# Shreyas2409/Rust-Image-Transform

Measured on AMD Instinct MI355X. Metric: transform MPix/s (decode+resize+encode) 4096²→512² WebP q80; 1/2/4/8 GPU, higher is better.
Workload: dtype u8

## Files before the change

rust-image-transform_amd/csrc/ik_inflate.h:

```cpp
#pragma once
#include <stdint.h>

#if defined(__HIPCC__) || defined(__HIP__)
#include <hip/hip_runtime.h>
#define IK_HD __host__ __device__ __forceinline__
#define IK_HD_COLD __host__ __device__ __attribute__((noinline))
#define IK_UNROLL _Pragma("unroll")
#else
#define IK_UNROLL
#define IK_HD inline
#define IK_HD_COLD inline
#endif

#if defined(__HIP_DEVICE_COMPILE__)
#define IK_GLOBAL __attribute__((address_space(1)))
#else
#define IK_GLOBAL
#endif

namespace ik {
namespace infl {

constexpr int kWindow = 32768;

// ... 391 lines not shown
        if (q < 0) return -1;
    }
    return -1;
}


constexpr int kCanonWords = 48;
struct CanonRegs {
    uint32_t lpk[8], dpk[8];
};
IK_HD void pack_limits(const uint32_t (&lim)[15], uint32_t (&pk)[8]) {
    for (int k = 0; k < 7; ++k)
        pk[k] = ((lim[2 * k] - 1u) & 0xFFFFu) | (((lim[2 * k + 1] - 1u) & 0xFFFFu) << 16);
    pk[7] = (lim[14] - 1u) & 0xFFFFu;
}

IK_HD uint32_t rev32(uint32_t v) {
#if defined(__HIP_DEVICE_COMPILE__)
    return __builtin_bitreverse32(v);
#else
    v = ((v >> 1) & 0x55555555u) | ((v & 0x55555555u) << 1);
    v = ((v >> 2) & 0x33333333u) | ((v & 0x33333333u) << 2);
    v = ((v >> 4) & 0x0F0F0F0Fu) | ((v & 0x0F0F0F0Fu) << 4);
    v = ((v >> 8) & 0x00FF00FFu) | ((v & 0x00FF00FFu) << 8);
    return (v >> 16) | (v << 16);
#endif
}

template <class Mem>
IK_HD uint8_t cm_byte(const Mem& m, int i) { return (uint8_t)(m[32 + (i >> 2)] >> (8 * (i & 3))); }

constexpr uint32_t kTokRaw = 0x4000u, kTokMatch = 0x8000u, kTokTable = 0xFFFFu, kTokPad = 0xFFFEu;
constexpr uint32_t kTokTableLen = 128;
constexpr uint32_t kTokSlack = 16;

IK_HD uint32_t tok_capacity(uint64_t bits, bool exact) {
    uint64_t c = (exact ? bits : bits / 4) + 2 * kTokTableLen + 64;
    if (c > 0x7FFFFFF0ull) c = 0x7FFFFFF0ull;
    return (uint32_t)((c + 7) & ~7ull);
}

struct TokOut {
    IK_GLOBAL uint16_t* p;
    uint64_t p0 = 0, p1 = 0, q0 = 0, q1 = 0;
    uint32_t ppos = 0, qpos = 0;
    int npend = 0;
    IK_HD void group(uint32_t pos, uint64_t lo, uint64_t hi) {
        if (npend == 0) {
            p0 = lo;
            p1 = hi;
            ppos = pos;
        } else {
            q0 = lo;
            q1 = hi;
            qpos = pos;
        }
        ++npend;
    }
    IK_HD void store1(uint32_t pos, uint64_t lo, uint64_t hi) {
#if defined(__HIP_DEVICE_COMPILE__)
        typedef uint32_t u4 __attribute__((ext_vector_type(4)));
        const u4 v = {(uint32_t)lo, (uint32_t)(lo >> 32), (uint32_t)hi, (uint32_t)(hi >> 32)};
        *reinterpret_cast<IK_GLOBAL u4*>(p + pos) = v;
#else
        for (int k = 0; k < 4; ++k) {
            p[pos + k] = (uint16_t)(lo >> (16 * k));
// ... 405 lines not shown
```

rust-image-transform_amd/csrc/ik_png.hip:

```cpp
#include <algorithm>
#include <cstdlib>
#include <cstring>
#include <type_traits>

#include "ik_crc.h"
#include "ik_inflate.h"
#include "ik_internal.h"
#include "ik_png.h"
#include "ik_png_wave.h"
#include "ik_unfilter.h"

namespace ik {

__device__ __forceinline__ void raise_priority() { __builtin_amdgcn_s_setprio(3); }

typedef __attribute__((address_space(3))) uint32_t lds_word;
struct FindWin {
    const IK_GLOBAL uint32_t* W;
    uint64_t wend;
    lds_word* win;
    uint32_t r0;
    __device__ void fetch(uint64_t base) {
        if (base + 32 > wend + 64) {
            for (int k = 0; k < 32; ++k) win[64 * k] = base + k < wend ? W[base + k] : 0u;
// ... 307 lines not shown
    }
    __device__ uint64_t operator()(uint32_t pos) {
        const uint32_t d = (pos >> 5) - wi;
        asm("" : "+v"(b0), "+v"(b1), "+v"(b2), "+v"(b3), "+v"(p0), "+v"(p1));
        const uint32_t n0 = d == 0 ? b0 : d == 1 ? b1 : b2;
        const uint32_t n1 = d == 0 ? b1 : d == 1 ? b2 : b3;
        const uint32_t n2 = d == 0 ? b2 : d == 1 ? b3 : p0;
        const uint32_t n3 = d == 0 ? b3 : d == 1 ? p0 : p1;
        b0 = n0;
        b1 = n1;
        b2 = n2;
        b3 = n3;
        wi += d;
        p0 = w[wi + 4];
        p1 = w[wi + 5];
        const uint32_t sh = pos & 31u;
        return ((uint64_t)__builtin_amdgcn_alignbit(b2, b1, sh) << 32) | __builtin_amdgcn_alignbit(b1, b0, sh);
    }
};
struct WaveGlobalWin {
    const IK_GLOBAL uint32_t* w;
    __device__ uint64_t operator()(uint64_t pos) const {
        const uint64_t wi = pos >> 5;
        const uint32_t sh = (uint32_t)(pos & 31u);
        const uint32_t a = w[wi], b = w[wi + 1], c = w[wi + 2];
        const uint32_t lo = __builtin_amdgcn_alignbit(b, a, sh), hi = __builtin_amdgcn_alignbit(c, b, sh);
        return ((uint64_t)hi << 32) | lo;
    }
};

struct WaveOut {
    IK_GLOBAL uint16_t* p;
    uint32_t cap;
    uint32_t n = 0;
    uint64_t g0 = 0, g1 = 0;
    __device__ void reset() { n = 0; g0 = 0; g1 = 0; }
    __device__ void mark(uint32_t, uint32_t) const {}
    __device__ void store(uint32_t g) const {
        if (g + 8u > cap) return;
        typedef uint32_t u4 __attribute__((ext_vector_type(4)));
        const u4 q = {(uint32_t)g0, (uint32_t)(g0 >> 32), (uint32_t)g1, (uint32_t)(g1 >> 32)};
        *reinterpret_cast<IK_GLOBAL u4*>(p + g) = q;
    }
    __device__ void put4(uint32_t a, uint32_t b, uint32_t c, uint32_t d, uint32_t k) {
        uint64_t T = (uint64_t)(a & 0xFFFFu) | ((uint64_t)(b & 0xFFFFu) << 16) | ((uint64_t)(c & 0xFFFFu) << 32) |
                     ((uint64_t)d << 48);
        T &= k >= 4u ? ~0ull : (1ull << (16u * k)) - 1ull;
        const uint32_t off = 16u * (n & 7u);
        const uint64_t lo_part = T << (off & 63u), hi_part = (T >> 1) >> (63u - (off & 63u));
        g0 |= off < 64u ? lo_part : 0ull;
        g1 |= off < 64u ? hi_part : lo_part;
        const uint64_t carry = off > 64u ? hi_part : 0ull;
        const uint32_t n2 = n + k;
        const bool done = ((n2 ^ n) & ~7u) != 0u;
        if (done) store(n & ~7u);
        g0 = done ? carry : g0;
        g1 = done ? 0ull : g1;
        n = n2;
    }
    __device__ void finish() {
        if (n & 7u) {
            constexpr uint64_t P = 0xFFFEFFFEFFFEFFFEull;
            const uint32_t off = 16u * (n & 7u);
            if (off < 64u) {
                g0 |= P << off;
                g1 |= P;
            } else {
                g1 |= P << (off - 64u);
            }
            store(n & ~7u);
        }
    }
};

__device__ __forceinline__ uint64_t shfl_up_u64(uint64_t v, int d) {
    const uint32_t lo = (uint32_t)__shfl_up((int)(uint32_t)v, d, 64), hi = (uint32_t)__shfl_up((int)(uint32_t)(v >> 32), d, 64);
    return ((uint64_t)hi << 32) | lo;
}
__device__ __forceinline__ uint64_t readlane_u64(uint64_t v, int l) {
    const uint32_t lo = (uint32_t)__builtin_amdgcn_readlane((int)(uint32_t)v, l);
    const uint32_t hi = (uint32_t)__builtin_amdgcn_readlane((int)(uint32_t)(v >> 32), l);
    return ((uint64_t)hi << 32) | lo;
}
__device__ __forceinline__ uint64_t wave_sum_u64(uint64_t v) {
#pragma unroll
    for (int o = 32; o >= 1; o >>= 1) {
        const uint32_t lo = (uint32_t)__shfl_xor((int)(uint32_t)v, o, 64), hi = (uint32_t)__shfl_xor((int)(uint32_t)(v >> 32), o, 64);
        v += ((uint64_t)hi << 32) | lo;
    }
    return v;
}

__device__ __forceinline__ uint32_t lane_rank(unsigned long long m) {
    return __builtin_amdgcn_mbcnt_hi((uint32_t)(m >> 32), __builtin_amdgcn_mbcnt_lo((uint32_t)m, 0u));
}

__device__ bool wave_code_build(const uint8_t* lens, int n, bool is_dist, bool fixed, wave::Code& C, uint16_t* syms) {
    const int lane = threadIdx.x;
    uint32_t cnt[16];
#pragma unroll
    for (int l = 0; l < 16; ++l) cnt[l] = 0;
    for (int c0 = 0; c0 < n; c0 += 64) {
        const int sy = c0 + lane;
// ... 414 lines not shown
        }
        if (bfinal) {
            final_block = 1;
            status = stop == ~0ull ? infl::kLaneOk : infl::kLaneMismatch;
            break;
        }
    }
    const uint32_t tsteps = (uint32_t)wave_sum_u64(steps);
    if (lane == 0) {
        infl::LaneResult r{};
        r.end_bit = p;
        r.out_len = total;
        r.ntok = (uint32_t)written;
        r.status = status;
        r.final_block = final_block;
        r.iters = tsteps;
        r.kcycles = (uint32_t)((clock64() - c0) >> 10);
        r.blocks = nblocks;
        r.pieces = npieces;
        r.kc_setup = (uint32_t)(ck_setup >> 10);
        r.units = nunits;
        res[t] = r;
#ifdef IK_WAVE_PROF
        wprof[0] = clock64() - c0;
        wprof[7] = 1;
        for (int k = 0; k < 8; ++k) atomicAdd(&g_wave_prof[k], (unsigned long long)wprof[k]);
#endif
    }
}

constexpr int kXRing = 2048;
constexpr int kXCap = 1024;
constexpr int kXNear = kXRing - kXCap;
using infl::kTokMatch;
using infl::kTokPad;
using infl::kTokRaw;
using infl::kTokTable;
using infl::kTokTableLen;

constexpr uint32_t kX8Tok = 512;
constexpr int kXFar = 64;
constexpr int kXPieces = 192;

#ifdef IK_EXP_PROF
__device__ unsigned long long g_exp_prof[8];
hipError_t png_exp_prof_read(unsigned long long* out) {
    hipError_t e = hipMemcpyFromSymbol(out, HIP_SYMBOL(g_exp_prof), sizeof(g_exp_prof));
    unsigned long long z[8] = {};
    if (e == hipSuccess) e = hipMemcpyToSymbol(HIP_SYMBOL(g_exp_prof), z, sizeof(z));
    return e;
}
#define IK_XP(k) do { const uint64_t _t = clock64(); xprof[k] += _t - xt; xt = _t; } while (0)
#else
#define IK_XP(k) ((void)0)
#endif

template <bool TAB>
__global__ __launch_bounds__(64) void k_png_expand8(const PngImgDev* imgs, const PngLaneDev* lanes, int nlanes,
                                                    const uint16_t* tok, int* status, const uint2* pieces,
                                                    const uint2* units, const uint32_t* ulane, PngMarks mk_out) {
    raise_priority();
    __shared__ __attribute__((aligned(16))) uint16_t s_ring[kXRing];
    __shared__ uint32_t s_tab[TAB ? 64 : 1];
    __shared__ uint32_t s_pb[kXPieces], s_ps[kXPieces];
    __shared__ uint32_t s_fo[kXFar], s_fd[kXFar], s_fc[kXFar];
    constexpr uint32_t M = kXRing - 1;
    typedef uint32_t u4 __attribute__((ext_vector_type(4)));
    const int li = blockIdx.x;
    if (li >= nlanes) return;
    const int x = threadIdx.x;
    const uint64_t c0 = clock64();
    const PngLaneDev L = lanes[units ? (int)ulane[li] : li];
    const PngImgDev I = imgs[L.img];
    const IK_GLOBAL uint16_t* T = (const IK_GLOBAL uint16_t*)(tok + L.tbase);
    IK_GLOBAL uint16_t* const U = (IK_GLOBAL uint16_t*)I.u16;
    int64_t ob = L.obase, oe = L.obase + (int64_t)L.out_len;
    uint32_t ntok = L.ntok;
    const uint32_t np = pieces ? L.npieces : 0u;
    const IK_GLOBAL uint2* P = (const IK_GLOBAL uint2*)(pieces + (pieces ? L.pbase : 0));
    uint32_t pf = 0, t0 = 0;
    if (units) {
        const IK_GLOBAL uint2* R = (const IK_GLOBAL uint2*)(units + L.pbase);
        const uint32_t b = (uint32_t)li - L.ubase;
        const uint2 r0 = make_uint2(R[b].x, R[b].y);
        const bool last = b + 1 >= L.nunits;
        uint2 r1 = make_uint2(np, (uint32_t)L.out_len);
        if (!last) r1 = make_uint2(R[b + 1].x, R[b + 1].y);
        pf = r0.x;
        t0 = P[pf].y;
        ntok = r1.x < np ? P[r1.x].y : L.ntok;
        ob = L.obase + (int64_t)r0.y;
        oe = L.obase + (int64_t)r1.y;
    }
    if (np) {
        for (uint32_t k = (uint32_t)x; pf + k < np && k < (uint32_t)kXPieces; k += 64) {
            s_pb[k] = P[pf + k].x;
            s_ps[k] = P[pf + k].y;
        }
        __syncthreads();
// ... 5 lines not shown
        pc_base = piece_base(pf);
        pn_start = pf + 1 < np ? piece_start(pf + 1) : 0xFFFFFFFFu;
    }
    uint32_t t = t0;
    int64_t cnt = 0;
    bool have_tab = false, bad = false;
    auto load8 = [&](uint32_t a) -> u4 {
        const uint32_t i = a + 8u * (uint32_t)x;
        if (i >= ntok) return u4{0xFFFEFFFEu, 0xFFFEFFFEu, 0xFFFEFFFEu, 0xFFFEFFFEu};
        if (!np) return *(const IK_GLOBAL u4*)(T + i);
        while (i >= pn_start) {
            ++kc;
            pc_base = piece_base(kc);
            pc_start = pn_start;
            pn_start = kc + 1 < np ? piece_start(kc + 1) : 0xFFFFFFFFu;
        }
        return *(const IK_GLOBAL u4*)(T + pc_base + (i - pc_start));
    };
    u4 w = load8(t0 & ~7u);
#ifdef IK_EXP_PROF
    uint64_t xprof[8] = {0, 0, 0, 0, 0, 0, 0, 0}, xt = clock64();
#endif
    while (t < ntok) {
        IK_XP(5);
        const uint32_t a = t & ~7u, i0 = a + 8u * (uint32_t)x;
        uint32_t u[8];
#pragma unroll
        for (int k = 0; k < 4; ++k) {
            u[2 * k] = w[k] & 0xFFFFu;
            u[2 * k + 1] = w[k] >> 16;
        }
        IK_XP(6);
        uint32_t end = a + kX8Tok < ntok ? a + kX8Tok : ntok;
        if constexpr (TAB) {
            int ft = 8;
#pragma unroll
            for (int k = 7; k >= 0; --k)
                if (i0 + k >= t && i0 + k < ntok && u[k] == kTokTable) ft = k;
            const unsigned long long tl = __ballot(ft < 8);
            if (tl) {
                const int l = __builtin_ctzll(tl);
                const uint32_t e = a + 8u * (uint32_t)l + (uint32_t)__builtin_amdgcn_readlane(ft, l);
                if (e == t) {
                    const uint32_t tt = (t + 8) & ~7u;
                    if (tt + kTokTableLen > ntok) { bad = true; break; }
                    s_tab[x] = ((const IK_GLOBAL uint32_t*)(T + tt))[x];
                    have_tab = true;
                    t = tt + kTokTableLen;
                    w = load8(t & ~7u);
                    __syncthreads();
                    continue;
                }
                end = e;
            }
        }
        {
            const uint32_t q = end - 1u;
            const bool mine = q >= t && (q >> 3) == (i0 >> 3);
            const uint32_t wq = w[(q >> 1) & 3u];
            const uint32_t uq = (q & 1u) ? wq >> 16 : wq & 0xFFFFu;
            if (__ballot(mine && (uq & 0xFF00u) == kTokMatch)) --end;
        }
        if (end <= t) { bad = true; break; }
        const uint32_t nx = (uint32_t)__shfl_down((int)u[0], 1, 64);
        const uint32_t pv = (uint32_t)__shfl_up((int)u[7], 1, 64);
        uint32_t len[8], val[8], lit = 0;
        uint32_t bd = 0;
#pragma unroll
        for (int k = 0; k < 8; ++k) {
            const uint32_t idx = i0 + k;
            const uint32_t prev = k ? u[k - 1] : pv, nxt = k < 7 ? u[k + 1] : nx;
            const uint32_t v = u[k];
            const bool start = (idx >= t) & (idx < end) & !((idx > t) & ((prev & 0xFF00u) == kTokMatch));
            const bool raw = (v & 0xFF00u) == kTokRaw, mt = (v & 0xFF00u) == kTokMatch, pad = v == kTokPad;
            const bool rk = TAB && v < 256u;
            const bool isl = raw | rk;
            len[k] = !start ? 0u : isl ? 1u : mt ? (v & 0xFFu) + 3u : 0u;
            uint32_t lv = v & 0xFFu;
            if constexpr (TAB) {
                if (start & rk) lv = (s_tab[v >> 2] >> (8 * (v & 3u))) & 0xFFu;
                bd |= (uint32_t)(start & rk & !have_tab);
            }
            val[k] = isl ? lv : nxt + 1u;
            lit |= (uint32_t)isl << k;
            bd |= (uint32_t)(start & !(isl | mt | pad));
        }
        if (__ballot(bd != 0u)) { bad = true; break; }
        uint32_t off[8], tot;
        for (;;) {
            uint32_t sum = 0;
#pragma unroll
            for (int k = 0; k < 8; ++k) sum += len[k];
            const uint32_t incl = wave_incl_scan_dpp(sum);
            tot = (uint32_t)__builtin_amdgcn_readlane((int)incl, 63);
            off[0] = incl - sum;
#pragma unroll
            for (int k = 1; k < 8; ++k) off[k] = off[k - 1] + len[k - 1];
            if (tot <= (uint32_t)kXCap) break;
            int fk = 8;
#pragma unroll
            for (int k = 7; k >= 0; --k)
                if (len[k] && off[k] + len[k] > (uint32_t)kXCap) fk = k;
            const unsigned long long ov = __ballot(fk < 8);
            const int l = __builtin_ctzll(ov);
            end = a + 8u * (uint32_t)l + (uint32_t)__builtin_amdgcn_readlane(fk, l);
#pragma unroll
            for (int k = 0; k < 8; ++k)
                if (i0 + k >= end) len[k] = 0;
        }
        IK_XP(1);
        const uint32_t t2 = end;
        const u4 wn = t2 < ntok ? load8(t2 & ~7u) : u4{0, 0, 0, 0};
        const uint32_t gb = (uint32_t)(ob + cnt);
#pragma unroll
        for (int k = 0; k < 8; ++k)
            if (len[k] && ((lit >> k) & 1u)) s_ring[(gb + off[k]) & M] = (uint16_t)val[k];
        uint32_t fcnt = 0, flen = 0;
#pragma unroll
        for (int k = 0; k < 8; ++k) {
            const bool fk = len[k] != 0u && !((lit >> k) & 1u) && val[k] > (uint32_t)kXNear;
            fcnt += fk ? 1u : 0u;
            flen += fk ? len[k] : 0u;
        }
        const uint32_t fp = fcnt | (flen << 16), fincl = wave_incl_scan_dpp(fp);
        const uint32_t ftot = (uint32_t)__builtin_amdgcn_readlane((int)fincl, 63);
        const uint32_t F = ftot & 0xFFFFu, FT = ftot >> 16;
        const bool flat = F != 0u && F <= (uint32_t)kXFar;
        if (flat) {
            uint32_t ri = (fincl - fp) & 0xFFFFu, rc = (fincl - fp) >> 16;
#pragma unroll
            for (int k = 0; k < 8; ++k) {
                const bool fk = len[k] != 0u && !((lit >> k) & 1u) && val[k] > (uint32_t)kXNear;
                if (fk) {
                    s_fo[ri] = off[k];
                    s_fd[ri] = val[k];
                    s_fc[ri] = rc;
                    ++ri;
                    rc += len[k];
                }
            }
            __syncthreads();
            for (uint32_t j = (uint32_t)x; j < FT; j += 64) {
                uint32_t m = 0;
                for (uint32_t q = 1; q < F; ++q) m = s_fc[q] <= j ? q : m;
                const uint32_t o = s_fo[m], d = s_fd[m], jj = j - s_fc[m];
                const int32_t sr = (int32_t)(o + jj) - (int32_t)d;
// ... 1058 lines not shown
```

rust-image-transform_amd/csrc/ik_png_decode.cpp:

```cpp
#include <hip/hip_runtime.h>

#include <algorithm>
#include <atomic>
#include <cassert>
#include <chrono>
#include <condition_variable>
#include <map>
#include <cstdio>
#include <memory>
#include <mutex>
#include <cmath>
#include <cstdlib>
#include <cstring>
#include <string>
#include <vector>

#include "../../include/imagekit_hip.h"
#include "ik_png.h"
#include "ik_png_plan.h"
#include "ik_png_wave.h"
#include "ik_runtime.h"

namespace ik {

// ... 790 lines not shown
    void rec(int k) { if (ev.ok) (void)hipEventRecord(ev.e[k], s); }
    void reject(PngJob& j, const char* why, bool no_room = false) {
        j.state = -1;
        j.suspect = !no_room;
        if (timing) fprintf(stderr, "[png] stream %d (%ux%u) -> host decoder: %s\n", j.idx, j.w, j.h, why);
    }
    void next_search(hipEvent_t after) {
        up.on_next_search(after);
        search_done = true;
    }
};

void png_plan_work(PngStage& T, PngWork& W, Xfer& X) {
    const bool wavedec = T.wavedec;
    Carver lay;
    W.M = T.m;
    for (PngJob* j : T.J) {
        size_t ftb = j->h;
        if (j->interlaced) {
            ftb = 0;
            for (int q = 0; q < j->npass; ++q) ftb += j->pass[q].ph;
            W.M += j->npass;
            ++W.n_il;
        }
        W.o_u16.push_back(lay.take<uint16_t>(j->raw_total + 64));
        W.o_ft.push_back(lay.take<uint8_t>(ftb));
    }
    for (PngJob* j : T.J) {
        W.max_lanes += (size_t)j->nchunks + (wavedec ? (size_t)j->nchunks / 4 + 16 : 0);
        W.tok_total += lane_tok_capacity(j->nbits, false) + (uint64_t)j->nchunks * (lane_tok_capacity(0, false) +
                                                                                    infl::kTokSlack);
    }
    W.tok_total += W.tok_total / 2 + 64;
    if (wavedec) {
        for (PngJob* j : T.J) W.pieces_total += wave::pieces_capacity(j->nbits) + 64ull * (uint64_t)j->nchunks;
        W.pieces_total += W.pieces_total / 2 + 4096;
    }
    for (PngJob* j : T.J) {
        W.npages += (j->raw_total >> kPngPageShift) + 1;
        for (int q = 0; q < (j->interlaced ? j->npass : 1); ++q) {
            const uint32_t hq = j->interlaced ? j->pass[q].ph : j->h;
            W.nrows += hq;
            W.nbands += ((size_t)hq + 63) / 64;
            W.ngroups += (size_t)png_unfilter_groups((int)hq);
        }
    }
    const size_t M = (size_t)W.M, max_lanes = W.max_lanes;
    lay.take(M, &W.d_imgs);
    lay.take(M, &W.d_err);
    lay.take(max_lanes, &W.d_lanes);
    lay.take(max_lanes, &W.d_res);
    lay.take(max_lanes, &W.d_obase);
    lay.take(2 * max_lanes, &W.d_xst);
    lay.take(max_lanes, &W.d_order);
    lay.take(M, &W.d_cls);
    lay.take(W.nrows, &W.d_rows);
    lay.take(W.npages, &W.d_pages);
    lay.take(W.ngroups, &W.d_groups);
    lay.take(M, &W.d_pbase);
    const size_t o_prog = lay.take(W.nbands + 8, &W.d_prog);
    W.unf_zero = lay.cur - o_prog;
    lay.take((size_t)W.n_il, &W.d_a7);
    lay.take(W.pieces_total, &W.d_pieces);
    lay.take(W.pieces_total, &W.d_units);
    lay.take(W.tok_total, &W.d_tok);
    W.dev = scratch_slot(2, lay.cur);
// ... 852 lines not shown
```

rust-image-transform_amd/csrc/ik_png_model.cpp:

```cpp
#include <cstdio>
#include <cstdlib>
#include <cstring>
#include <map>
#include <vector>

#include "ik_crc.h"
#include "ik_inflate.h"
#include "ik_png_gather.h"
#include "ik_png_plan.h"
#include "ik_png_wave.h"
#include "ik_unfilter.h"

using namespace ik;

namespace {
struct HostWin {
    const uint32_t* W;
    uint64_t wend;
    uint32_t w[32];
    void fetch(uint64_t base) {
        for (int k = 0; k < 32; ++k) w[k] = base + k < wend ? W[base + k] : 0u;
    }
    uint32_t word(uint32_t k) const { return w[k]; }
};
// ... 125 lines not shown
    stats[8] = overflows;
    stats[2] = (int)L.start.size();
    stats[3] = L.rounds;
    stats[5] = (int)(nl0 - L.start.size());
    stats[7] = st;
    if (st) return -2;
    std::vector<int64_t> obase;
    uint64_t total;
    pngplan::offsets(L, obase, &total);
    if (total > out_cap) return -3;
    std::vector<uint16_t> u16(total + 16);
    for (size_t i = 0; i < L.start.size(); ++i) {
        infl::TokInHost tin{tok[i].data()};
        if (infl::expand_lane(tin, L.res[i].ntok, infl::U16Out{u16.data()}, obase[i], L.res[i].out_len)) return -4;
    }
    const int shift = 12;
    std::vector<int> pages((total >> shift) + 1);
    for (size_t pg = 0, ln = 0; pg < pages.size(); ++pg) {
        while (ln + 1 < obase.size() && (uint64_t)obase[ln + 1] <= (pg << shift)) ++ln;
        pages[pg] = (int)ln;
    }
    int markers = 0;
    for (uint64_t q = 0; q < total; ++q) {
        if (u16[q] >= 256) ++markers;
        const int v = infl::resolve_at(u16.data(), obase.data(), (int)obase.size(), pages.data(), shift, (int64_t)q);
        if (v < 0) return -5;
        out[q] = (uint8_t)v;
    }
    stats[4] = markers;
    *out_len = total;
    return 0;
}

int ikm_inflate_wave(const uint8_t* z, size_t zlen, size_t chunk_bytes, uint8_t* out, size_t out_cap,
                     uint64_t* out_len, uint64_t* stats) {
    for (int i = 0; i < 20; ++i) stats[i] = 0;
    if (const char* e = getenv("IKM_EST")) {
        long a = 1024, b = 4096, c = 16384;
        if (sscanf(e, "%ld,%ld,%ld", &a, &b, &c) == 3) { wave::g_est_mul = a; wave::g_est_add = b; wave::g_min_tail = c; }
    }
    if (zlen < 2) return -1;
    if ((z[0] & 15) != 8 || ((z[0] << 8) | z[1]) % 31 || (z[1] & 0x20)) return -1;
    const uint64_t nbits = (uint64_t)zlen * 8;
    std::vector<uint32_t> words((zlen + 3) / 4 + 8, 0);
    std::memcpy(words.data(), z, zlen);
    std::vector<int64_t> cand;
    const int found = find_candidates(words, nbits, chunk_bytes, cand);
    if (found < 0) return found;
    stats[0] = cand.size();
    stats[1] = (uint64_t)found;
    struct W {
        const uint32_t* words;
        uint64_t nw;
        uint64_t operator()(uint64_t pos) const {
            const uint64_t wi = pos >> 5;
            const uint32_t sh = (uint32_t)(pos & 31);
            auto rd = [&](uint64_t i) -> uint64_t { return i < nw ? words[i] : 0u; };
            const uint64_t lo = rd(wi) | (rd(wi + 1) << 32);
            return sh ? (lo >> sh) | (rd(wi + 2) << (64 - sh)) : lo;
        }
    } win{words.data(), (nbits >> 5) + 1};
    pngplan::Lanes L;
    pngplan::build(cand, L);
    std::map<uint64_t, std::vector<uint16_t>> tok;
    std::map<uint64_t, std::vector<std::pair<uint32_t, uint32_t>>> pieces;
    std::map<uint64_t, std::vector<std::pair<uint32_t, uint32_t>>> units;
    wave::Stats ws;
    int st, overflows = 0;
    for (;;) {
// ... 37 lines not shown
    stats[6] = ws.sub_passes;
    stats[7] = ws.redo_passes;
    stats[8] = ws.fix_rounds;
    stats[9] = ws.max_rounds;
    stats[10] = ws.blocks;
    stats[11] = ws.symbols_bits;
    stats[12] = (uint64_t)(int64_t)st;
    stats[15] = ws.steps;
    stats[16] = ws.wave_steps;
    if (getenv("IKM_PROF"))
        fprintf(stderr, "[model] first-pass wave steps %llu: any slow literal %.1f%%, slow distance %.1f%%, group store "
                "%.1f%%, match %.1f%%, warm-up %.1f%%\n", (unsigned long long)ws.prof[7],
                100.0 * ws.prof[0] / ws.prof[7], 100.0 * ws.prof[1] / ws.prof[7], 100.0 * ws.prof[2] / ws.prof[7],
                100.0 * ws.prof[3] / ws.prof[7], 100.0 * ws.prof[4] / ws.prof[7]);
    if (st) return -2;
    std::vector<int64_t> obase;
    uint64_t total;
    pngplan::offsets(L, obase, &total);
    if (total > out_cap) return -3;
    std::vector<uint16_t> u16(total + 16);
    std::vector<int64_t> uob;
    for (size_t i = 0; i < L.start.size(); ++i) {
        const std::vector<std::pair<uint32_t, uint32_t>>& pt = pieces[L.start[i]];
        const std::vector<std::pair<uint32_t, uint32_t>>& ut = units[L.start[i]];
        const std::vector<uint16_t>& t = tok[L.start[i]];
        if (ut.empty() && L.res[i].out_len) return -4;
        for (size_t u = 0; u < ut.size(); ++u) {
            const uint32_t p0 = ut[u].first, p1 = u + 1 < ut.size() ? ut[u + 1].first : (uint32_t)pt.size();
            const uint64_t o0 = ut[u].second, o1 = u + 1 < ut.size() ? ut[u + 1].second : L.res[i].out_len;
            if (p0 > p1 || p1 > pt.size() || o0 > o1) return -4;
            std::vector<uint16_t> cat;
            for (uint32_t k = p0; k < p1; ++k) {
                const uint32_t n = (k + 1 < pt.size() ? pt[k + 1].second : L.res[i].ntok) - pt[k].second;
                cat.insert(cat.end(), t.begin() + pt[k].first, t.begin() + pt[k].first + n);
            }
            stats[13] += cat.size();
            stats[17] += 1;
            for (size_t q = 0; q + 1 < cat.size(); ++q) {
                const uint32_t v = cat[q];
                if ((v & 0xFF00u) != infl::kTokMatch) continue;
                const uint32_t len = (v & 255u) + 3, d = (uint32_t)cat[q + 1] + 1;
                stats[d <= 1024 ? 18 : 19] += 1;
                if (getenv("IKM_PROF")) {
                    static uint64_t hist[8] = {0};
                    hist[d <= 4 ? 0 : d <= 64 ? 1 : d <= 1024 ? 2 : d <= 16384 ? 3 : d <= 16388 ? 4 : 5] += 1;
                    hist[6] += len;
                    hist[7] += 1;
                    if ((hist[7] & ((1u << 16) - 1)) == 0)
                        fprintf(stderr, "[model] matches %llu: d<=4 %llu, <=64 %llu, <=1024 %llu, <=16384 %llu, 16385-16388 %llu, "
                                "farther %llu; mean length %.1f\n", (unsigned long long)hist[7], (unsigned long long)hist[0],
                                (unsigned long long)hist[1], (unsigned long long)hist[2], (unsigned long long)hist[3],
                                (unsigned long long)hist[4], (unsigned long long)hist[5], (double)hist[6] / hist[7]);
                }
                ++q;
            }
            cat.resize(cat.size() + 16, (uint16_t)infl::kTokPad);
            infl::TokInHost tin{cat.data()};
            const int64_t ob = obase[i] + (int64_t)o0;
            uob.push_back(ob);
            if (infl::expand_lane(tin, (uint32_t)(cat.size() - 16), infl::U16Out{u16.data()}, ob, o1 - o0)) {
                if (getenv("IKM_DEBUG"))
                    fprintf(stderr, "lane %zu unit %zu/%zu expand failed: tokens %zu, out %llu\n", i, u, ut.size(),
                            cat.size() - 16, (unsigned long long)(o1 - o0));
                return -4;
            }
        }
    }
    obase.swap(uob);
    const int shift = 12;
// ... 189 lines not shown
```

rust-image-transform_amd/csrc/ik_png_wave.h:

```cpp
#pragma once
#include <stdint.h>

#include "ik_inflate.h"

namespace ik {
namespace wave {

#if defined(__HIP_DEVICE_COMPILE__)
#define IK_KEEP(x, y) asm volatile("" ::"v"(x), "v"(y))
#else
#define IK_KEEP(x, y) ((void)0)
#endif

constexpr int kLB = 10;
constexpr int kDB = 8;
constexpr uint32_t kLM = (1u << kLB) - 1u, kDM = (1u << kDB) - 1u;
constexpr int kSub = 64;
constexpr int kWarmBits = 256;
constexpr int kMinSubBits = 512;
#ifndef IK_WAVE_WINDOW_BYTES
#define IK_WAVE_WINDOW_BYTES 10496
#endif
constexpr uint64_t kWindowBits = 8ull * IK_WAVE_WINDOW_BYTES;
static_assert(kWindowBits % 128 == 0, "windows are staged in 16-byte groups");

enum { kKLit = 0, kKLen = 1, kKEob = 2, kKSlow = 3 };
IK_HD uint32_t e_bits(uint32_t e) { return e & 31u; }
IK_HD uint32_t e_kind(uint32_t e) { return (e >> 5) & 3u; }
IK_HD bool e_two(uint32_t e) { return (e >> 7) & 1u; }
IK_HD uint32_t e_lit1(uint32_t e) { return (e >> 8) & 255u; }
IK_HD uint32_t e_lit2(uint32_t e) { return (e >> 16) & 255u; }
IK_HD uint32_t e_len1(uint32_t e) { return (e >> 24) & 15u; }
IK_HD uint32_t e_lextra(uint32_t e) { return (e >> 8) & 7u; }
IK_HD uint32_t e_lbase(uint32_t e) { return ((e >> 16) & 255u) + 3u; }
// ... 95 lines not shown
        if (s2 >= 0 && s2 < 256 && L2 <= (int)r) return mk_lit2((uint32_t)L, (uint32_t)s, (uint32_t)L2, (uint32_t)s2);
    }
    return lit_symbol_entry(s, (uint32_t)L);
}
template <class CodeT, class Syms>
IK_HD uint32_t dist_table_entry(uint32_t e, const CodeT& C, const Syms& syms) {
    int D;
    const int s = canon_sym(e, C, syms, D);
    if (D > kDB || s < 0) return kSlowDist;
    return dist_symbol_entry(s, (uint32_t)D);
}

template <class Syms>
IK_HD uint32_t lit_slow(uint64_t v, const Code& C, const Syms& syms) {
    int L;
    const int s = canon_sym((uint32_t)v & 0x7FFFu, C, syms, L);
    if (s < 0) return kSlowEntry;
    return lit_symbol_entry(s, (uint32_t)L);
}
template <class Syms>
IK_HD uint32_t dist_slow(uint64_t v, const Code& C, const Syms& syms) {
    int D;
    const int s = canon_sym((uint32_t)v & 0x7FFFu, C, syms, D);
    if (s < 0) return kSlowDist;
    return dist_symbol_entry(s, (uint32_t)D);
}

struct SubOutHost {
    uint16_t* p;
    uint32_t cap;
    uint32_t n = 0;
    uint8_t* marks = nullptr;
    uint32_t nmarks = 0;
    IK_HD void reset() { n = 0; }
    IK_HD void mark(uint32_t step, uint32_t f) {
        if (marks && step - 1 < nmarks) marks[step - 1] |= (uint8_t)f;
    }
    IK_HD void put4(uint32_t a, uint32_t b, uint32_t c, uint32_t d, uint32_t k) {
        const uint32_t t[4] = {a, b, c, d};
        for (uint32_t i = 0; i < k; ++i) {
            if (n < cap) p[n] = (uint16_t)t[i];
            ++n;
        }
    }
    IK_HD void finish() {
        for (uint32_t i = n; i < ((n + 7u) & ~7u); ++i)
            if (i < cap) p[i] = (uint16_t)infl::kTokPad;
    }
};

struct SubRes {
    uint32_t start;
    uint32_t exit;
    uint32_t out;
    uint32_t ntok;
    int eob;
    int bad;
    int over;
    uint32_t steps;
};

template <class Win, class LitTab, class DistTab, class LSyms, class DSyms, class Out>
IK_HD void sub_decode(Win& win, uint32_t p0, uint32_t lo, uint32_t hi, const LitTab& lit, const DistTab& dist,
                      const Code& LC, const LSyms& lsyms, const Code& DC, const DSyms& dsyms, Out& out,
                      SubRes& r) {
    uint32_t pos = p0;
    win.init(p0);
    r.start = p0 >= lo ? p0 : ~0u;
    r.eob = 0;
    r.bad = 0;
    out.reset();
    uint32_t cnt = 0;
    uint32_t steps = 0;
    bool stop = pos >= hi;
    while (!stop) {
        ++steps;
        const bool started = pos >= lo;
        r.start = (started & (r.start == ~0u)) ? pos : r.start;
        const uint32_t limit = started ? hi : lo;
        const uint64_t v = win(pos);
        uint32_t e1 = lit[(uint32_t)v & kLM];
        const bool slow1 = e_kind(e1) == kKSlow;
        if (slow1) e1 = lit_slow(v, LC, lsyms);
        const uint32_t k1 = e_kind(e1), n1 = e_bits(e1), L1 = e_len1(e1);
        const bool isl = k1 == kKLit;
        const bool two1 = e_two(e1) & (pos + L1 < limit);
        const uint32_t c1 = two1 ? n1 : L1;
        const uint32_t e2 = lit[(uint32_t)(v >> c1) & kLM];
        const bool lit2 = ((uint32_t)isl & ((uint32_t)two1 | (uint32_t)!e_two(e1)) & (uint32_t)(pos + c1 < limit) &
                           (uint32_t)(e_kind(e2) == kKLit)) != 0u;
        const uint32_t L2 = e_len1(e2);
        const bool two2 = lit2 & e_two(e2) & (pos + c1 + L2 < limit);
        const uint32_t c2 = lit2 ? (two2 ? e_bits(e2) : L2) : 0u;
        const uint32_t le = e_lextra(e1);
        const uint32_t ll = e_lbase(e1) + ((uint32_t)(v >> n1) & ((1u << le) - 1u));
        const uint64_t vd = v >> (n1 + le);
        uint32_t d = dist[(uint32_t)vd & kDM];
        const bool isn = k1 == kKLen;
        const bool slow2 = isn & d_slow(d);
        if (slow2) d = dist_slow(vd, DC, dsyms);
        const bool bad = (k1 == kKSlow) | (isn & d_slow(d));
        const uint32_t D = d_len(d), de = d_extra(d);
        const uint32_t dd = d_base(d) + ((uint32_t)(vd >> D) & ((1u << de) - 1u));
        IK_KEEP(ll, dd);
        const bool eob = k1 == kKEob;
        const bool fin = started & (bad | eob);
        const uint32_t t1 = isl ? infl::kTokRaw | e_lit1(e1) : infl::kTokMatch | (ll - 3u);
        const uint32_t t2l = infl::kTokRaw | (two1 ? e_lit2(e1) : e_lit1(e2)), t2m = dd - 1u;
        IK_KEEP(t2l, t2m);
        const uint32_t t2 = isl ? t2l : t2m;
        const uint32_t t3 = infl::kTokRaw | (two1 ? e_lit1(e2) : e_lit2(e2));
        const uint32_t t4 = infl::kTokRaw | e_lit2(e2);
        const uint32_t nl = 1u + (two1 ? 1u : 0u) + (lit2 ? 1u : 0u) + (two2 ? 1u : 0u);
        const bool emit = started & !fin;
        const uint32_t k = !emit ? 0u : isl ? nl : isn ? 2u : 0u;
        out.mark(steps, (slow1 ? 1u : 0u) | (slow2 ? 2u : 0u) | (((out.n + k) ^ out.n) & ~7u ? 4u : 0u) |
                            (isn ? 8u : 0u) | (!started ? 16u : 0u));
        out.put4(t1, t2, t3, t4, k);
        cnt += !emit ? 0u : isl ? nl : isn ? ll : 0u;
        const uint32_t adv_l = c1 + c2, adv_n = n1 + le + D + de;
        IK_KEEP(adv_l, adv_n);
        const uint32_t adv = isl ? adv_l : isn ? adv_n : eob ? n1 : 1u;
        pos += (fin & bad) ? 0u : adv;
        r.eob = fin & eob;
        r.bad = fin & bad;
        stop = fin | (pos >= hi);
    }
    if (r.start == ~0u) r.start = pos;
    r.exit = pos;
    r.out = cnt;
    r.ntok = out.n;
    r.over = ((out.n + 7u) & ~7u) > out.cap;
    r.steps = steps;
}

IK_HD uint32_t pieces_capacity(uint64_t bits) {
    const uint64_t c = bits / 512 + 64;
    return (uint32_t)(c < (1u << 24) ? c : (1u << 24));
}

struct Split {
    int nsub;
    uint32_t lw;
    uint32_t cap;
};
IK_HD Split split_range(uint64_t bp, uint64_t re, bool big) {
    const uint64_t bits = re > bp ? re - bp : 1;
    uint64_t ns = bits / kMinSubBits;
    ns = ns < 1 ? 1 : ns > (uint64_t)kSub ? (uint64_t)kSub : ns;
    uint64_t lw = (bits + 32 * ns - 1) / (32 * ns);
    lw |= 1u;
    ns = (bits + 32 * lw - 1) / (32 * lw);
    Split s;
    s.nsub = (int)(ns < 1 ? 1 : ns);
    s.lw = (uint32_t)lw;
    const uint64_t c = (big ? 32 * lw : 12 * lw) + 32;
    s.cap = (uint32_t)((c + 7) & ~7ull);
    return s;
}
#if !defined(__HIP_DEVICE_COMPILE__)
inline int64_t g_est_mul = 1024, g_est_add = 4096, g_min_tail = 16384;
#endif
IK_HD uint64_t block_end_estimate(uint64_t body, uint64_t prev_bits) {
#if !defined(__HIP_DEVICE_COMPILE__)
    return prev_bits ? body + prev_bits * (uint64_t)g_est_mul / 1024 + (uint64_t)g_est_add : 0;
#else
    return prev_bits ? body + prev_bits + 4096 : 0;
#endif
}
IK_HD uint64_t window_end(uint64_t bp, uint64_t stop_eff, uint64_t est_end) {
    uint64_t re = bp + kWindowBits < stop_eff ? bp + kWindowBits : stop_eff;
    if (est_end) {
#if !defined(__HIP_DEVICE_COMPILE__)
        const uint64_t e = est_end > bp + (uint64_t)g_min_tail ? est_end : bp + (uint64_t)g_min_tail;
#else
        const uint64_t e = est_end > bp + 16384 ? est_end : bp + 16384;
#endif
        if (e < re) re = e;
    }
    return re;
}

IK_HD uint64_t region_capacity(uint64_t bits, bool big) {
    const uint64_t slack = (bits / kWindowBits + 2) * (48ull * kSub) + 64;
    const uint64_t c = big ? bits + 32ull * pieces_capacity(bits) + slack : bits / 8 * 3 + slack;
    return (c + 7) & ~7ull;
}

struct Stats {
    uint64_t windows = 0, sub_passes = 0, redo_passes = 0, fix_rounds = 0, max_rounds = 0;
    uint64_t symbols_bits = 0, blocks = 0, slow = 0, steps = 0;
    uint64_t wave_steps = 0;
    uint64_t prof[8] = {0, 0, 0, 0, 0, 0, 0, 0};
};

#ifndef IK_UNIT_MIN_TOK
#define IK_UNIT_MIN_TOK 16384
#endif
constexpr uint32_t kUnitMinTok = IK_UNIT_MIN_TOK;
IK_HD bool unit_starts(uint32_t nunits, uint64_t written, uint64_t unit_v0) {
    return nunits == 0 || written - unit_v0 >= kUnitMinTok;
}

#if !defined(__HIP_DEVICE_COMPILE__)
template <class WinFn, class Pieces>
inline void lane_host(WinFn win, uint64_t nbits, uint64_t start, uint64_t stop, bool big, uint16_t* region,
                      uint64_t cap, infl::LaneResult& r, Pieces& pt, Pieces& units, Stats* stats,
                      uint64_t warm = kWarmBits) {
    const uint32_t pcap = pieces_capacity((stop == ~0ull ? nbits : stop) - start);
    const uint64_t stop_eff = stop == ~0ull ? nbits : stop;
    uint64_t p = start, used = 0, total = 0, written = 0;
    uint64_t prev_bits = 0;
    r.status = infl::kLaneCorrupt;
    r.final_block = 0;
    r.blocks = 0;
    r.iters = 0;
    pt.clear();
    units.clear();
// ... 124 lines not shown
                        redo[j] = j > v && !sr[j - 1].eob && !sr[j - 1].bad && sr[j].start != sr[j - 1].exit;
                    }
                    uint32_t redo_max = 0;
                    for (int j = v + 1; j < sp.nsub; ++j) {
                        if (!redo[j]) continue;
                        SubOutHost o{region + used + (uint64_t)j * sp.cap, sp.cap};
                        sub_decode(rwin, ex[j - 1], lo[j], lo[j + 1], lit, dist, LC, lsyms, DC, dsyms, o, sr[j]);
                        o.finish();
                        if (stats) { ++stats->redo_passes; stats->steps += sr[j].steps; }
                        redo_max = sr[j].steps > redo_max ? sr[j].steps : redo_max;
                    }
                    if (stats) stats->wave_steps += redo_max;
                }
                if (stats) {
                    stats->fix_rounds += (uint64_t)rounds;
                    if ((uint64_t)rounds > stats->max_rounds) stats->max_rounds = (uint64_t)rounds;
                }
                bool over = false;
                for (int j = 0; j <= v; ++j) over = over || sr[j].over;
                if (over) {
                    r.status = infl::kLaneOverflow;
                    done = 3;
                    break;
                }
                if (pt.size() + (size_t)(v + 1) > pcap) {
                    r.status = blk_start > start ? (int)infl::kLaneSplit : (int)infl::kLaneOverflow;
                    done = 4;
                    break;
                }
#ifdef IKM_WAVE_DEBUG
                for (int j = 0; j <= v; ++j) {
                    const uint16_t* q = region + used + (uint64_t)j * sp.cap;
                    uint64_t nb = 0;
                    for (uint32_t k = 0; k < ((sr[j].ntok + 7u) & ~7u); ++k) {
                        const uint32_t t = q[k];
                        if ((t & 0xFF00u) == infl::kTokRaw) ++nb;
                        else if ((t & 0xFF00u) == infl::kTokMatch) { nb += (t & 255u) + 3; ++k; }
                    }
                    if (nb != sr[j].out)
                        fprintf(stderr, "sub-lane %d of %d: tokens %u describe %llu bytes, counted %llu (start %llu exit %llu lo %llu hi %llu eob %d)\n",
                                j, sp.nsub, sr[j].ntok, (unsigned long long)nb, (unsigned long long)sr[j].out,
                                (unsigned long long)sr[j].start, (unsigned long long)sr[j].exit, (unsigned long long)lo[j],
                                (unsigned long long)lo[j + 1], sr[j].eob);
                }
#endif
                for (int j = 0; j <= v; ++j) {
                    pt.push_back({(uint32_t)(used + (uint64_t)j * sp.cap), (uint32_t)written});
                    written += (sr[j].ntok + 7u) & ~7u;
                    total += sr[j].out;
                    if (stats) stats->symbols_bits += sr[j].exit - sr[j].start;
                }
                used += (uint64_t)v * sp.cap + ((sr[v].ntok + 7u) & ~7u);
                if (sr[v].bad) { done = 3; break; }
                if (sr[v].eob) {
                    p = bp + sr[v].exit;
                    prev_bits = p - body;
                    done = 1;
                    break;
                }
                bp += sr[v].exit;
            }
            if (done == 4) {
                pt.resize(blk_pieces);
                units.resize(blk_units);
                unit_v0 = blk_v0;
                total = blk_total;
                used = blk_used;
                written = blk_written;
// ... 21 lines not shown
```

Measured before the change: 31750.

## Pack literal runs into byte-packed token groups in wave inflate output

New measurement: 29890. 5.9% lower.

```diff
diff --git a/rust-image-transform_amd/csrc/ik_inflate.h b/rust-image-transform_amd/csrc/ik_inflate.h
--- a/rust-image-transform_amd/csrc/ik_inflate.h
+++ b/rust-image-transform_amd/csrc/ik_inflate.h
@@ -447,6 +447,7 @@
 
 constexpr uint32_t kTokRaw = 0x4000u, kTokMatch = 0x8000u, kTokTable = 0xFFFFu, kTokPad = 0xFFFEu;
 constexpr uint32_t kTokTableLen = 128;
+constexpr uint32_t kTokLitTag = 0xC0u, kTokLitMax = 15;
 constexpr uint32_t kTokSlack = 16;
 
 IK_HD uint32_t tok_capacity(uint64_t bits, bool exact) {
diff --git a/rust-image-transform_amd/csrc/ik_png.hip b/rust-image-transform_amd/csrc/ik_png.hip
--- a/rust-image-transform_amd/csrc/ik_png.hip
+++ b/rust-image-transform_amd/csrc/ik_png.hip
@@ -363,43 +363,63 @@
 struct WaveOut {
     IK_GLOBAL uint16_t* p;
     uint32_t cap;
-    uint32_t n = 0;
+    uint32_t st = 0;
     uint64_t g0 = 0, g1 = 0;
-    __device__ void reset() { n = 0; g0 = 0; g1 = 0; }
+    __device__ void reset() { st = 0; g0 = 0; g1 = 0; }
     __device__ void mark(uint32_t, uint32_t) const {}
-    __device__ void store(uint32_t g) const {
-        if (g + 8u > cap) return;
+    __device__ uint32_t total() const { return ((st >> 5) + ((st & 15u) ? 1u : 0u)) << 3; }
+    __device__ void store(uint64_t lo, uint64_t hi) const {
+        const uint32_t n = (st >> 5) << 3;
+        if (n + 8u > cap) return;
         typedef uint32_t u4 __attribute__((ext_vector_type(4)));
-        const u4 q = {(uint32_t)g0, (uint32_t)(g0 >> 32), (uint32_t)g1, (uint32_t)(g1 >> 32)};
-        *reinterpret_cast<IK_GLOBAL u4*>(p + g) = q;
-    }
-    __device__ void put4(uint32_t a, uint32_t b, uint32_t c, uint32_t d, uint32_t k) {
-        uint64_t T = (uint64_t)(a & 0xFFFFu) | ((uint64_t)(b & 0xFFFFu) << 16) | ((uint64_t)(c & 0xFFFFu) << 32) |
-                     ((uint64_t)d << 48);
-        T &= k >= 4u ? ~0ull : (1ull << (16u * k)) - 1ull;
-        const uint32_t off = 16u * (n & 7u);
-        const uint64_t lo_part = T << (off & 63u), hi_part = (T >> 1) >> (63u - (off & 63u));
+        const u4 q = {(uint32_t)lo, (uint32_t)(lo >> 32), (uint32_t)hi, (uint32_t)(hi >> 32)};
+        *reinterpret_cast<IK_GLOBAL u4*>(p + n) = q;
+    }
+    __device__ bool put(uint32_t B, uint32_t M, uint32_t kl, bool km) {
+        constexpr uint64_t kTag = (uint64_t)infl::kTokLitTag << 56;
+        const uint32_t off = (st & 15u) << 3;
+        const bool m = off ? ((st >> 4) & 1u) != 0u : km;
+        const bool ff = km & !m;
+        const uint64_t L16 = (uint64_t)__builtin_amdgcn_perm(0x40404040u, B, 0x05010400u) |
+                             ((uint64_t)__builtin_amdgcn_perm(0x40404040u, B, 0x05030402u) << 32);
+        uint64_t T = km ? (uint64_t)M : m ? L16 : (uint64_t)B;
+        const uint32_t wd = km ? 32u : m ? 16u * kl : 8u * kl;
+        T &= wd >= 64u ? ~0ull : (1ull << wd) - 1ull;
+        const uint32_t end = ff ? off : m ? 128u : 120u;
+        const uint64_t Ta = ff ? 0ull : T;
+        const uint64_t lo_part = Ta << (off & 63u), hi_part = (Ta >> 1) >> (63u - (off & 63u));
         g0 |= off < 64u ? lo_part : 0ull;
         g1 |= off < 64u ? hi_part : lo_part;
-        const uint64_t carry = off > 64u ? hi_part : 0ull;
-        const uint32_t n2 = n + k;
-        const bool done = ((n2 ^ n) & ~7u) != 0u;
-        if (done) store(n & ~7u);
+        const uint32_t off2 = off + wd;
+        const bool done = (wd != 0u) & (off2 >= end);
+        const uint64_t tag = kTag | ((uint64_t)(ff ? off >> 3 : infl::kTokLitMax) << 56);
+        const uint64_t g1s = (ff | !m) ? (g1 & 0x00FFFFFFFFFFFFFFull) | tag : g1;
+        if (done) store(g0, g1s);
+        const uint32_t sh = end - off;
+        const uint64_t carry = sh >= 64u ? 0ull : T >> sh;
         g0 = done ? carry : g0;
         g1 = done ? 0ull : g1;
-        n = n2;
+        st = ((st >> 5) + (done ? 1u : 0u)) << 5 | ((m | ff) ? 16u : 0u) | ((done ? off2 - end : off2) >> 3);
+        return done;
     }
     __device__ void finish() {
-        if (n & 7u) {
-            constexpr uint64_t P = 0xFFFEFFFEFFFEFFFEull;
-            const uint32_t off = 16u * (n & 7u);
-            if (off < 64u) {
-                g0 |= P << off;
-                g1 |= P;
+        const uint32_t off = (st & 15u) << 3;
+        if (off) {
+            if ((st >> 4) & 1u) {
+                constexpr uint64_t P = 0xFFFEFFFEFFFEFFFEull;
+                if (off < 64u) {
+                    g0 |= P << off;
+                    g1 |= P;
+                } else {
+                    g1 |= P << (off - 64u);
+                }
             } else {
-                g1 |= P << (off - 64u);
-            }
-            store(n & ~7u);
+                g1 |= (uint64_t)(infl::kTokLitTag | (off >> 3)) << 56;
+            }
+            store(g0, g1);
+            st = ((st >> 5) + 1u) << 5;
+            g0 = 0;
+            g1 = 0;
         }
     }
 };
@@ -880,6 +900,8 @@
 constexpr int kXRing = 2048;
 constexpr int kXCap = 1024;
 constexpr int kXNear = kXRing - kXCap;
+constexpr int kXCapLit = kXCap - 16;
+static_assert(kXCapLit + 14 + kXNear <= kXRing && kXNear >= kXCap, "the ring holds a batch, its overshoot and the near sources");
 using infl::kTokMatch;
 using infl::kTokPad;
 using infl::kTokRaw;
@@ -913,6 +935,7 @@
     __shared__ uint32_t s_pb[kXPieces], s_ps[kXPieces];
     __shared__ uint32_t s_fo[kXFar], s_fd[kXFar], s_fc[kXFar];
     constexpr uint32_t M = kXRing - 1;
+    constexpr uint32_t kCap = TAB ? kXCap : kXCapLit;
     typedef uint32_t u4 __attribute__((ext_vector_type(4)));
     const int li = blockIdx.x;
     if (li >= nlanes) return;
@@ -984,6 +1007,15 @@
         }
         IK_XP(6);
         uint32_t end = a + kX8Tok < ntok ? a + kX8Tok : ntok;
+        bool lg = false, lgbad = false;
+        uint32_t nl = 0;
+        if constexpr (!TAB) {
+            lg = (w[3] >> 28) == (infl::kTokLitTag >> 4);
+            nl = lg ? (w[3] >> 24) & 15u : 0u;
+            lgbad = lg & ((nl == 0u) | (i0 < t));
+#pragma unroll
+            for (int k = 0; k < 8; ++k) u[k] = lg ? kTokPad : u[k];
+        }
         if constexpr (TAB) {
             int ft = 8;
 #pragma unroll
@@ -1011,7 +1043,7 @@
             const bool mine = q >= t && (q >> 3) == (i0 >> 3);
             const uint32_t wq = w[(q >> 1) & 3u];
             const uint32_t uq = (q & 1u) ? wq >> 16 : wq & 0xFFFFu;
-            if (__ballot(mine && (uq & 0xFF00u) == kTokMatch)) --end;
+            if (__ballot(mine && !lg && (uq & 0xFF00u) == kTokMatch)) --end;
         }
         if (end <= t) { bad = true; break; }
         const uint32_t nx = (uint32_t)__shfl_down((int)u[0], 1, 64);
@@ -1037,10 +1069,11 @@
             lit |= (uint32_t)isl << k;
             bd |= (uint32_t)(start & !(isl | mt | pad));
         }
-        if (__ballot(bd != 0u)) { bad = true; break; }
+        if (__ballot((bd != 0u) | lgbad)) { bad = true; break; }
+        nl = i0 < end ? nl : 0u;
         uint32_t off[8], tot;
         for (;;) {
-            uint32_t sum = 0;
+            uint32_t sum = nl;
 #pragma unroll
             for (int k = 0; k < 8; ++k) sum += len[k];
             const uint32_t incl = wave_incl_scan_dpp(sum);
@@ -1048,22 +1081,36 @@
             off[0] = incl - sum;
 #pragma unroll
             for (int k = 1; k < 8; ++k) off[k] = off[k - 1] + len[k - 1];
-            if (tot <= (uint32_t)kXCap) break;
+            if (tot <= kCap) break;
             int fk = 8;
 #pragma unroll
             for (int k = 7; k >= 0; --k)
-                if (len[k] && off[k] + len[k] > (uint32_t)kXCap) fk = k;
+                if (len[k] && off[k] + len[k] > kCap) fk = k;
+            if (nl && off[0] + nl > kCap) fk = 0;
             const unsigned long long ov = __ballot(fk < 8);
             const int l = __builtin_ctzll(ov);
             end = a + 8u * (uint32_t)l + (uint32_t)__builtin_amdgcn_readlane(fk, l);
 #pragma unroll
             for (int k = 0; k < 8; ++k)
                 if (i0 + k >= end) len[k] = 0;
+            nl = i0 < end ? nl : 0u;
         }
         IK_XP(1);
         const uint32_t t2 = end;
         const u4 wn = t2 < ntok ? load8(t2 & ~7u) : u4{0, 0, 0, 0};
         const uint32_t gb = (uint32_t)(ob + cnt);
+        if constexpr (!TAB) {
+            if (__ballot(nl != 0u)) {
+                if (nl) {
+                    const uint32_t rb = gb + off[0];
+#pragma unroll
+                    for (int k = 14; k >= 0; --k) {
+                        s_ring[(rb + (uint32_t)k) & M] = (uint16_t)((w[k >> 2] >> (8 * (k & 3))) & 0xFFu);
+                        asm volatile("" ::: "memory");
+                    }
+                }
+            }
+        }
 #pragma unroll
         for (int k = 0; k < 8; ++k)
             if (len[k] && ((lit >> k) & 1u)) s_ring[(gb + off[k]) & M] = (uint16_t)val[k];
diff --git a/rust-image-transform_amd/csrc/ik_png_decode.cpp b/rust-image-transform_amd/csrc/ik_png_decode.cpp
--- a/rust-image-transform_amd/csrc/ik_png_decode.cpp
+++ b/rust-image-transform_amd/csrc/ik_png_decode.cpp
@@ -846,6 +846,14 @@
                                                                                     infl::kTokSlack);
     }
     W.tok_total += W.tok_total / 2 + 64;
+    {
+        uint64_t big1 = 0;
+        for (PngJob* j : T.J) {
+            const uint64_t c = lane_tok_capacity(j->nbits < (1ull << 20) ? j->nbits : (1ull << 20), true) + infl::kTokSlack;
+            big1 = c > big1 ? c : big1;
+        }
+        W.tok_total += big1;
+    }
     if (wavedec) {
         for (PngJob* j : T.J) W.pieces_total += wave::pieces_capacity(j->nbits) + 64ull * (uint64_t)j->nchunks;
         W.pieces_total += W.pieces_total / 2 + 4096;
diff --git a/rust-image-transform_amd/csrc/ik_png_model.cpp b/rust-image-transform_amd/csrc/ik_png_model.cpp
--- a/rust-image-transform_amd/csrc/ik_png_model.cpp
+++ b/rust-image-transform_amd/csrc/ik_png_model.cpp
@@ -181,9 +181,17 @@
     return 0;
 }
 
+int ikm_inflate_wave_pieces(const uint8_t* z, size_t zlen, size_t chunk_bytes, uint8_t* out, size_t out_cap,
+                            uint64_t* out_len, uint64_t* stats, uint32_t* rec, size_t rec_cap, uint64_t* nrec);
 int ikm_inflate_wave(const uint8_t* z, size_t zlen, size_t chunk_bytes, uint8_t* out, size_t out_cap,
                      uint64_t* out_len, uint64_t* stats) {
+    return ikm_inflate_wave_pieces(z, zlen, chunk_bytes, out, out_cap, out_len, stats, nullptr, 0, nullptr);
+}
+
+int ikm_inflate_wave_pieces(const uint8_t* z, size_t zlen, size_t chunk_bytes, uint8_t* out, size_t out_cap,
+                            uint64_t* out_len, uint64_t* stats, uint32_t* rec, size_t rec_cap, uint64_t* nrec) {
     for (int i = 0; i < 20; ++i) stats[i] = 0;
+    if (nrec) *nrec = 0;
     if (const char* e = getenv("IKM_EST")) {
         long a = 1024, b = 4096, c = 16384;
         if (sscanf(e, "%ld,%ld,%ld", &a, &b, &c) == 3) { wave::g_est_mul = a; wave::g_est_add = b; wave::g_min_tail = c; }
@@ -287,9 +295,37 @@
             std::vector<uint16_t> cat;
             for (uint32_t k = p0; k < p1; ++k) {
                 const uint32_t n = (k + 1 < pt.size() ? pt[k + 1].second : L.res[i].ntok) - pt[k].second;
-                cat.insert(cat.end(), t.begin() + pt[k].first, t.begin() + pt[k].first + n);
-            }
-            stats[13] += cat.size();
+                if ((uint64_t)pt[k].first + n > t.size()) return -4;
+                const size_t c0 = cat.size();
+                uint64_t gc[3] = {0, 0, 0};
+                if (!wave::unpack_groups(t.data() + pt[k].first, n, cat, gc)) return -4;
+                stats[13] += n;
+                if (nrec) {
+                    uint64_t ob = 0;
+                    bool last_match = false;
+                    for (size_t q = c0; q < cat.size(); ++q) {
+                        const uint32_t v = cat[q];
+                        if ((v & 0xFF00u) == infl::kTokRaw) { ++ob; last_match = false; }
+                        else if ((v & 0xFF00u) == infl::kTokMatch) { ob += (v & 255u) + 3; ++q; last_match = true; }
+                    }
+                    const uint32_t tag = n >= 8 ? t[pt[k].first + 7] >> 8 : 0u;
+                    const uint32_t first = (tag & 0xF0u) == infl::kTokLitTag ? tag & 15u : 0u;
+                    if (*nrec < rec_cap) {
+                        uint32_t* r = rec + 10 * *nrec;
+                        r[0] = (uint32_t)i;
+                        r[1] = k;
+                        r[2] = pt[k].first;
+                        r[3] = pt[k].second;
+                        r[4] = n;
+                        r[5] = L.res[i].ntok;
+                        r[6] = (uint32_t)ob;
+                        r[7] = (uint32_t)gc[0];
+                        r[8] = (uint32_t)gc[1];
+                        r[9] = first | (k == p0 ? 0x100u : 0u) | (last_match ? 0x200u : 0u);
+                    }
+                    ++*nrec;
+                }
+            }
             stats[17] += 1;
             for (size_t q = 0; q + 1 < cat.size(); ++q) {
                 const uint32_t v = cat[q];
diff --git a/rust-image-transform_amd/csrc/ik_png_wave.h b/rust-image-transform_amd/csrc/ik_png_wave.h
--- a/rust-image-transform_amd/csrc/ik_png_wave.h
+++ b/rust-image-transform_amd/csrc/ik_png_wave.h
@@ -1,5 +1,7 @@
 #pragma once
 #include <stdint.h>
+
+#include <vector>
 
 #include "ik_inflate.h"
 
@@ -161,22 +163,94 @@
     uint32_t n = 0;
     uint8_t* marks = nullptr;
     uint32_t nmarks = 0;
-    IK_HD void reset() { n = 0; }
-    IK_HD void mark(uint32_t step, uint32_t f) {
+    uint32_t fill = 0;
+    bool u16 = false;
+    uint8_t g[16] = {0, 0, 0, 0, 0, 0, 0, 0, 0, 0, 0, 0, 0, 0, 0, 0};
+    void reset() {
+        n = 0;
+        fill = 0;
+        u16 = false;
+        for (int i = 0; i < 16; ++i) g[i] = 0;
+    }
+    void mark(uint32_t step, uint32_t f) {
         if (marks && step - 1 < nmarks) marks[step - 1] |= (uint8_t)f;
     }
-    IK_HD void put4(uint32_t a, uint32_t b, uint32_t c, uint32_t d, uint32_t k) {
-        const uint32_t t[4] = {a, b, c, d};
-        for (uint32_t i = 0; i < k; ++i) {
-            if (n < cap) p[n] = (uint16_t)t[i];
-            ++n;
-        }
-    }
-    IK_HD void finish() {
-        for (uint32_t i = n; i < ((n + 7u) & ~7u); ++i)
-            if (i < cap) p[i] = (uint16_t)infl::kTokPad;
+    uint32_t total() const { return n + (fill ? 8u : 0u); }
+    void close() {
+        if (!u16) g[15] = (uint8_t)(infl::kTokLitTag | fill);
+        if (n + 8u <= cap)
+            for (int i = 0; i < 8; ++i) p[n + i] = (uint16_t)(g[2 * i] | (g[2 * i + 1] << 8));
+        n += 8;
+        fill = 0;
+        for (int i = 0; i < 16; ++i) g[i] = 0;
+    }
+    bool slot(uint32_t v) {
+        g[2 * fill] = (uint8_t)v;
+        g[2 * fill + 1] = (uint8_t)(v >> 8);
+        if (++fill < 8u) return false;
+        close();
+        return true;
+    }
+    bool put(uint32_t B, uint32_t M, uint32_t kl, bool km) {
+        bool stored = false;
+        bool m = fill ? u16 : km;
+        if (km && !m) {
+            close();
+            stored = true;
+            m = true;
+        }
+        u16 = m;
+        if (km) {
+            stored |= slot(M & 0xFFFFu);
+            stored |= slot(M >> 16);
+            return stored;
+        }
+        for (uint32_t i = 0; i < kl; ++i) {
+            const uint32_t b = (B >> (8 * i)) & 255u;
+            if (m) {
+                stored |= slot(infl::kTokRaw | b);
+            } else {
+                g[fill] = (uint8_t)b;
+                if (++fill == infl::kTokLitMax) {
+                    close();
+                    stored = true;
+                }
+            }
+        }
+        return stored;
+    }
+    void finish() {
+        if (!fill) return;
+        if (u16)
+            for (uint32_t i = fill; i < 8; ++i) {
+                g[2 * i] = (uint8_t)infl::kTokPad;
+                g[2 * i + 1] = (uint8_t)(infl::kTokPad >> 8);
+            }
+        close();
     }
 };
+
+#if !defined(__HIP_DEVICE_COMPILE__)
+inline bool unpack_groups(const uint16_t* in, size_t nslots, std::vector<uint16_t>& out, uint64_t* counts = nullptr) {
+    for (size_t q = 0; q + 8 <= nslots; q += 8) {
+        const uint32_t tag = in[q + 7] >> 8;
+        if ((tag & 0xF0u) == infl::kTokLitTag) {
+            const uint32_t n = tag & 15u;
+            if (n == 0) return false;
+            for (uint32_t i = 0; i < n; ++i)
+                out.push_back((uint16_t)(infl::kTokRaw | ((in[q + (i >> 1)] >> (8 * (i & 1u))) & 255u)));
+            if (counts) {
+                ++counts[0];
+                counts[1] += n < infl::kTokLitMax;
+            }
+        } else {
+            out.insert(out.end(), in + q, in + q + 8);
+            if (counts) ++counts[2];
+        }
+    }
+    return nslots % 8 == 0;
+}
+#endif
 
 struct SubRes {
     uint32_t start;
@@ -234,18 +308,14 @@
         IK_KEEP(ll, dd);
         const bool eob = k1 == kKEob;
         const bool fin = started & (bad | eob);
-        const uint32_t t1 = isl ? infl::kTokRaw | e_lit1(e1) : infl::kTokMatch | (ll - 3u);
-        const uint32_t t2l = infl::kTokRaw | (two1 ? e_lit2(e1) : e_lit1(e2)), t2m = dd - 1u;
-        IK_KEEP(t2l, t2m);
-        const uint32_t t2 = isl ? t2l : t2m;
-        const uint32_t t3 = infl::kTokRaw | (two1 ? e_lit1(e2) : e_lit2(e2));
-        const uint32_t t4 = infl::kTokRaw | e_lit2(e2);
+        const uint32_t a1 = (e1 >> 8) & 0xFFFFu, a2 = (e2 >> 8) & 0xFFFFu;
+        const uint32_t B = two1 ? a1 | (a2 << 16) : (a1 & 0xFFu) | (a2 << 8);
+        const uint32_t M = (infl::kTokMatch | (ll - 3u)) | ((dd - 1u) << 16);
         const uint32_t nl = 1u + (two1 ? 1u : 0u) + (lit2 ? 1u : 0u) + (two2 ? 1u : 0u);
         const bool emit = started & !fin;
-        const uint32_t k = !emit ? 0u : isl ? nl : isn ? 2u : 0u;
-        out.mark(steps, (slow1 ? 1u : 0u) | (slow2 ? 2u : 0u) | (((out.n + k) ^ out.n) & ~7u ? 4u : 0u) |
-                            (isn ? 8u : 0u) | (!started ? 16u : 0u));
-        out.put4(t1, t2, t3, t4, k);
+        const bool stored = out.put(B, M, (emit & isl) ? nl : 0u, emit & isn);
+        out.mark(steps, (slow1 ? 1u : 0u) | (slow2 ? 2u : 0u) | (stored ? 4u : 0u) | (isn ? 8u : 0u) |
+                            (!started ? 16u : 0u));
         cnt += !emit ? 0u : isl ? nl : isn ? ll : 0u;
         const uint32_t adv_l = c1 + c2, adv_n = n1 + le + D + de;
         IK_KEEP(adv_l, adv_n);
@@ -258,8 +328,8 @@
     if (r.start == ~0u) r.start = pos;
     r.exit = pos;
     r.out = cnt;
-    r.ntok = out.n;
-    r.over = ((out.n + 7u) & ~7u) > out.cap;
+    r.ntok = out.total();
+    r.over = out.total() > out.cap;
     r.steps = steps;
 }
 
@@ -283,7 +353,7 @@
     Split s;
     s.nsub = (int)(ns < 1 ? 1 : ns);
     s.lw = (uint32_t)lw;
-    const uint64_t c = (big ? 32 * lw : 12 * lw) + 32;
+    const uint64_t c = big ? 64 * lw + 128 : 8 * lw + 32;
     s.cap = (uint32_t)((c + 7) & ~7ull);
     return s;
 }
@@ -311,8 +381,8 @@
 }
 
 IK_HD uint64_t region_capacity(uint64_t bits, bool big) {
-    const uint64_t slack = (bits / kWindowBits + 2) * (48ull * kSub) + 64;
-    const uint64_t c = big ? bits + 32ull * pieces_capacity(bits) + slack : bits / 8 * 3 + slack;
+    const uint64_t slack = (bits / kWindowBits + 2) * ((big ? 224ull : 48ull) * kSub) + 64;
+    const uint64_t c = big ? 2 * bits + 256ull * pieces_capacity(bits) + slack : bits / 4 + slack;
     return (c + 7) & ~7ull;
 }
 
@@ -503,8 +573,10 @@
                 for (int j = 0; j <= v; ++j) {
                     const uint16_t* q = region + used + (uint64_t)j * sp.cap;
                     uint64_t nb = 0;
-                    for (uint32_t k = 0; k < ((sr[j].ntok + 7u) & ~7u); ++k) {
-                        const uint32_t t = q[k];
+                    std::vector<uint16_t> uq;
+                    unpack_groups(q, (sr[j].ntok + 7u) & ~7u, uq);
+                    for (size_t k = 0; k < uq.size(); ++k) {
+                        const uint32_t t = uq[k];
                         if ((t & 0xFF00u) == infl::kTokRaw) ++nb;
                         else if ((t & 0xFF00u) == infl::kTokMatch) { nb += (t & 255u) + 3; ++k; }
                     }
```
